# soedinglab/hh-suite

Measured on NVIDIA H100. Metric: Viterbi GCUPS (query_L x sum target_L / s), higher is better.
Workload: dtype f32

## Files before the change

### hh-suite_b200/csrc/hhg_api.cu

```cuda
#include "../../include/hhg.h"
#include "hhg_kernels.cuh"
#include "hhg_hhm.cuh"
#include "hhg_msa.cuh"
#include "hhg_crf.cuh"
#include "hhg_mac.cuh"
#include "hhg_topk.cuh"
#include "hhg_hitlist.h"

#include <dlfcn.h>
#if defined(__SSE__)
#include <xmmintrin.h>
#endif

#include <algorithm>
#include <chrono>
#include <atomic>
#include <cstdarg>
#include <cstdio>
#include <cstdlib>
#include <cstring>
#include <memory>
#include <cmath>
#include <cfloat>
#include <mutex>
// ... 1377 lines not shown
int hhg_set_use_ss(hhg_ctx* ctx, int use_ss) {
  if (!ctx) return fail(HHG_EINVAL, "ctx is NULL");
  if (use_ss && (!ctx->has_ss || !ctx->has_S33)) return fail(HHG_EINVAL, "hhg_set_use_ss: the query was set without ss / S33");
  ctx->par.use_ss = use_ss ? 1 : 0;
  return HHG_OK;
}

static int plan_strip_rows(const hhg_ctx* ctx, const int32_t* req_query, int n) {
  if (ctx->R) return ctx->R;
  long long items16 = 0;
  if (!req_query) items16 = (long long)((n + 31) / 32) * ((ctx->q_L[0] + 15) / 16);
  else {
    std::vector<long long> cnt(ctx->nq, 0);
    for (int k = 0; k < n; ++k) if (req_query[k] >= 0 && req_query[k] < ctx->nq) cnt[req_query[k]]++;
    for (int q = 0; q < ctx->nq; ++q) items16 += (cnt[q] + 31) / 32 * ((ctx->q_L[q] + 15) / 16);
  }
  return items16 >= 4LL * ctx->sm_count * 8 ? 16 : 8;
}

static int plan_build(hhg_ctx* ctx, hhg_plan* pl, const hhg_db* db, int n, const int32_t* ids,
                      const int32_t* req_query = nullptr) {
  if (!ctx || !db || n <= 0) return fail(HHG_EINVAL, "hhg_plan_create: bad argument");
  if (ctx->nq <= 0) return fail(HHG_EINVAL, "hhg_plan_create: no query set");
  if (db->device != ctx->device) return fail(HHG_EINVAL, "db lives on device %d, ctx on %d", db->device, ctx->device);
  CK(cudaSetDevice(ctx->device));
  const int R = plan_strip_rows(ctx, req_query, n);
  if (pl->db == db && pl->db_serial == db->serial && pl->n == n && pl->R == R && pl->q_L == ctx->q_L &&
      pl->q_row0 == ctx->q_row0 && !pl->ids.empty() && pl->max_bt_bytes == ctx->max_bt_bytes) {
    bool same = true;
    if (ids) same = memcmp(ids, pl->ids.data(), (size_t)n * 4) == 0;
    else for (int k = 0; k < n && same; ++k) same = pl->ids[k] == k;
    if (same) {
      if (req_query) same = memcmp(req_query, pl->req_query.data(), (size_t)n * 4) == 0;
      else for (int k = 0; k < n && same; ++k) same = pl->req_query[k] == 0;
    }
    if (same) { pl->celloff = false; return HHG_OK; }
  }
  pl->db = db;
  pl->db_serial = db->serial;
  pl->device = db->device;
  pl->max_bt_bytes = ctx->max_bt_bytes;
  pl->cells = pl->padded_cells = pl->alg_bytes = 0;
  pl->waves.clear();
  pl->celloff = false;
  pl->n = n;
  pl->R = R;
  pl->q_L = ctx->q_L; pl->q_row0 = ctx->q_row0;
  pl->Lq = ctx->q_L[0];
  pl->ids.resize(n); pl->req_query.resize(n);
  for (int k = 0; k < n; ++k) {
    const int id = ids ? ids[k] : k;
    if (id < 0 || id >= db->n) return fail(HHG_EINVAL, "request %d: target id %d out of range", k, id);
    const int q = req_query ? req_query[k] : 0;
    if (q < 0 || q >= ctx->nq) return fail(HHG_EINVAL, "request %d: query index %d out of range (batch of %d)", k, q, ctx->nq);
    pl->ids[k] = id; pl->req_query[k] = q;
  }
  pl->order.resize(n);
  std::iota(pl->order.begin(), pl->order.end(), 0);
  std::stable_sort(pl->order.begin(), pl->order.end(), [&](int a, int b) {
    if (pl->req_query[a] != pl->req_query[b]) return pl->req_query[a] < pl->req_query[b];
    return db->L[pl->ids[a]] > db->L[pl->ids[b]];
  });
  std::vector<int> job_first, job_cnt;
  for (int k = 0; k < n;) {
    const int q = pl->req_query[pl->order[k]];
    int e = k;
    while (e < n && e - k < 32 && pl->req_query[pl->order[e]] == q) ++e;
    job_first.push_back(k); job_cnt.push_back(e - k);
    k = e;
  }
  pl->njobs = (int)job_first.size();
  pl->req_job.resize(n); pl->req_lane.resize(n);
  pl->job_Lmax.resize(pl->njobs); pl->job_query.resize(pl->njobs); pl->job_nstrips.resize(pl->njobs);
  pl->job_Lq.resize(pl->njobs); pl->job_qrow0.resize(pl->njobs); pl->job_ss_off.resize(pl->njobs);
  pl->job_bt_off.resize(pl->njobs); pl->job_bnd_off.resize(pl->njobs); pl->job_co_off.resize(pl->njobs);
  pl->job_jc_off.resize(pl->njobs);
  pl->jc_version = 0;
  std::vector<int> job_target((size_t)pl->njobs * 32);
  std::vector<int> req_Lt(n), req_Lq(n);
  long long bnd = 0, co = 0, jc = 0, ss = 0;
  size_t wave_bt = 0, max_wave_words = 0;
  Wave w;
  for (int jb = 0; jb < pl->njobs; ++jb) {
    const int first = job_first[jb], cnt = job_cnt[jb];
    const int q = pl->req_query[pl->order[first]];
    const int Lmax = db->L[pl->ids[pl->order[first]]];
    const int ns = (ctx->q_L[q] + R - 1) / R;
    pl->job_Lmax[jb] = Lmax; pl->job_query[jb] = q; pl->job_nstrips[jb] = ns;
    pl->job_Lq[jb] = ctx->q_L[q]; pl->job_qrow0[jb] = ctx->q_row0[q];
    for (int l = 0; l < 32; ++l) {
      const int rq = pl->order[first + std::min(l, cnt - 1)];
      job_target[(size_t)jb * 32 + l] = pl->ids[rq];
      if (l < cnt) { pl->req_job[rq] = jb; pl->req_lane[rq] = l; }
    }
    const size_t words = (size_t)(ns * R / 4) * (Lmax + 1) * 32;
    if (wave_bt > 0 && (wave_bt + words) * 4 > ctx->max_bt_bytes) {
      w.job_end = jb;
      pl->waves.push_back(w);
      max_wave_words = std::max(max_wave_words, wave_bt);
      w.job_begin = jb;
      wave_bt = 0;
    }
    pl->job_bt_off[jb] = (long long)wave_bt;
    wave_bt += words;
    pl->job_bnd_off[jb] = bnd;
    bnd += (long long)(Lmax + 1) * 32;
    pl->job_co_off[jb] = co;
    pl->job_jc_off[jb] = jc;
    pl->job_ss_off[jb] = ss;
    jc += (long long)Lmax * 224;
    co += (long long)ns * (Lmax + 1) * 32;
    ss += ns;
    pl->padded_cells += (double)ns * R * (double)Lmax * 32.0;
  }
  w.job_end = pl->njobs;
  pl->waves.push_back(w);
  max_wave_words = std::max(max_wave_words, wave_bt);
  pl->ss_total = ss;
  pl->co_total = co;
  pl->items.clear();
  for (Wave& wv : pl->waves) {
    wv.item_begin = (long long)pl->items.size();
    for (int g0 = wv.job_begin; g0 < wv.job_end; g0 += ctx->group_jobs) {
      const int g1 = std::min(g0 + ctx->group_jobs, wv.job_end);
      int maxns = 0;
      for (int jb = g0; jb < g1; ++jb) maxns = std::max(maxns, pl->job_nstrips[jb]);
      for (int sidx = 0; sidx < maxns; ++sidx)
        for (int jb = g0; jb < g1; ++jb)
          if (sidx < pl->job_nstrips[jb]) pl->items.push_back(make_int2(jb - wv.job_begin, sidx));
    }
    wv.item_end = (long long)pl->items.size();
  }
  pl->path_off.resize(n);
  long long po = 0;
  double cols_sum = 0;
  for (int k = 0; k < n; ++k) {
    const int Lt = db->L[pl->ids[k]];
    const int Lqk = ctx->q_L[pl->req_query[k]];
    req_Lt[k] = Lt; req_Lq[k] = Lqk;
    pl->path_off[k] = po;
    po += Lqk + Lt + 2;
    pl->cells += (double)Lqk * Lt;
    cols_sum += Lt;
  }
  if (po > 0x7fffffffLL) return fail(HHG_EINVAL, "plan too large: %lld path bytes (> 2^31-1); split the request", po);
  pl->path_total = po;
  pl->jc_total = jc;
  pl->alg_bytes = cols_sum * 112.0 + pl->cells * 1.0 + (double)sizeof(HitRec) * n;

  cudaError_t e = cudaSuccess;
  auto A = [&](cudaError_t r) { if (e == cudaSuccess) e = r; };
  A(pl->d_job_target.ensure(job_target.size())); A(pl->d_job_Lmax.ensure(pl->njobs));
  A(pl->d_job_bt_off.ensure(pl->njobs)); A(pl->d_job_bnd_off.ensure(pl->njobs)); A(pl->d_job_co_off.ensure(pl->njobs));
  A(pl->d_job_jc_off.ensure(pl->njobs)); A(pl->d_jcols.ensure((size_t)jc + 224));
  A(pl->d_job_query.ensure(pl->njobs)); A(pl->d_job_nstrips.ensure(pl->njobs)); A(pl->d_job_Lq.ensure(pl->njobs));
  A(pl->d_job_qrow0.ensure(pl->njobs)); A(pl->d_job_ss_off.ensure(pl->njobs)); A(pl->d_items.ensure(pl->items.size()));
  A(pl->d_req_job.ensure(n)); A(pl->d_req_lane.ensure(n)); A(pl->d_req_Lt.ensure(n)); A(pl->d_req_Lq.ensure(n));
  A(pl->d_path_off.ensure(n));
  A(pl->d_req_target.ensure(n)); A(pl->d_S.ensure((size_t)po));
  A(pl->d_bt.ensure(max_wave_words));
  { BndSlot* before = pl->d_bnd.p; A(pl->d_bnd.ensure((size_t)bnd + 32));
    if (e == cudaSuccess && pl->d_bnd.p != before) A(cudaMemsetAsync(pl->d_bnd.p, 0, pl->d_bnd.n * sizeof(BndSlot), ctx->stream)); }
  A(pl->d_strip_score.ensure((size_t)ss * 32));
  A(pl->d_strip_ij.ensure((size_t)ss * 32));
  A(pl->d_counter.ensure(pl->waves.size()));
  A(pl->d_hits.ensure(n));
  A(pl->d_paths.ensure((size_t)po));
  if (e != cudaSuccess) return fail(HHG_ENOMEM, "hhg_plan_create: %s", cudaGetErrorString(e));

  cudaStream_t st = ctx->stream;
  auto H2D = [&](void* d, const void* h, size_t bytes) { return cudaMemcpyAsync(d, h, bytes, cudaMemcpyHostToDevice, st); };
  CK(H2D(pl->d_job_target.p, job_target.data(), job_target.size() * 4));
  CK(H2D(pl->d_job_Lmax.p, pl->job_Lmax.data(), (size_t)pl->njobs * 4));
  CK(H2D(pl->d_job_bt_off.p, pl->job_bt_off.data(), (size_t)pl->njobs * 8));
  CK(H2D(pl->d_job_bnd_off.p, pl->job_bnd_off.data(), (size_t)pl->njobs * 8));
  CK(H2D(pl->d_job_co_off.p, pl->job_co_off.data(), (size_t)pl->njobs * 8));
  CK(H2D(pl->d_job_jc_off.p, pl->job_jc_off.data(), (size_t)pl->njobs * 8));
  CK(H2D(pl->d_job_query.p, pl->job_query.data(), (size_t)pl->njobs * 4));
  CK(H2D(pl->d_job_nstrips.p, pl->job_nstrips.data(), (size_t)pl->njobs * 4));
  CK(H2D(pl->d_job_Lq.p, pl->job_Lq.data(), (size_t)pl->njobs * 4));
  CK(H2D(pl->d_job_qrow0.p, pl->job_qrow0.data(), (size_t)pl->njobs * 4));
  CK(H2D(pl->d_job_ss_off.p, pl->job_ss_off.data(), (size_t)pl->njobs * 8));
  CK(H2D(pl->d_items.p, pl->items.data(), pl->items.size() * sizeof(int2)));
  CK(H2D(pl->d_req_job.p, pl->req_job.data(), (size_t)n * 4));
  CK(H2D(pl->d_req_lane.p, pl->req_lane.data(), (size_t)n * 4));
  CK(H2D(pl->d_req_Lt.p, req_Lt.data(), (size_t)n * 4));
  CK(H2D(pl->d_req_Lq.p, req_Lq.data(), (size_t)n * 4));
  CK(H2D(pl->d_req_target.p, pl->ids.data(), (size_t)n * 4));
  CK(H2D(pl->d_path_off.p, pl->path_off.data(), (size_t)n * 8));
  CK(cudaStreamSynchronize(st));
  return HHG_OK;
}

int hhg_plan_create(hhg_ctx* ctx, const hhg_db* db, int n, const int32_t* ids, hhg_plan** out) {
  if (!out) return fail(HHG_EINVAL, "hhg_plan_create: out is NULL");
  std::unique_ptr<hhg_plan> pl(new hhg_plan());
  int rc = plan_build(ctx, pl.get(), db, n, ids);
  if (rc != HHG_OK) return rc;
  *out = pl.release();
  return HHG_OK;
}

int hhg_plan_destroy(hhg_plan* plan) {
  if (plan) { if (plan->db) cudaSetDevice(plan->device); delete plan; }
  return HHG_OK;
}
double hhg_plan_cells(const hhg_plan* plan) { return plan ? plan->cells : 0; }
double hhg_plan_padded_cells(const hhg_plan* plan) { return plan ? plan->padded_cells : 0; }
double hhg_plan_algorithmic_bytes(const hhg_plan* plan) { return plan ? plan->alg_bytes : 0; }

static int set_exclusions(hhg_ctx* ctx, hhg_plan* pl, const int64_t* excl_off, const int32_t* excl_i,
                          const int32_t* excl_j) {
  pl->celloff = false;
  pl->n_excl_steps = 0;
  const long long total = excl_off ? excl_off[pl->n] : 0;
  const bool regions = !ctx->ex_q_lo.empty() || !ctx->ex_t_lo.empty();
  if (total <= 0 && !regions) return HHG_OK;
  const size_t co_words = (size_t)pl->co_total;
  CK(pl->d_co.ensure(co_words));
  CK(cudaMemsetAsync(pl->d_co.p, 0, co_words * 4, ctx->stream));
  if (total > 0) {
    if (excl_off[0] != 0) return fail(HHG_EINVAL, "excl_off[0] must be 0");
    if (!excl_i || !excl_j) return fail(HHG_EINVAL, "excl_i / excl_j are NULL");
    std::vector<int> sreq((size_t)total);
    for (int k = 0; k < pl->n; ++k) {
      if (excl_off[k + 1] < excl_off[k]) return fail(HHG_EINVAL, "excl_off is not monotonic at request %d", k);
      const int Lt = pl->db->L[pl->ids[k]];
      for (long long s = excl_off[k]; s < excl_off[k + 1]; ++s) {
        const int Lqk = pl->q_L[pl->req_query[k]];
        if (excl_i[s] < 1 || excl_i[s] > Lqk || excl_j[s] < 1 || excl_j[s] > Lt)
          return fail(HHG_EINVAL, "excluded step %lld of request %d is (%d,%d), outside 1..%d x 1..%d", s - excl_off[k], k,
                      excl_i[s], excl_j[s], Lqk, Lt);
        sreq[(size_t)s] = k;
      }
    }
    CK(pl->d_step_req.ensure((size_t)total)); CK(pl->d_step_i.ensure((size_t)total)); CK(pl->d_step_j.ensure((size_t)total));
    CK(cudaMemcpyAsync(pl->d_step_req.p, sreq.data(), (size_t)total * 4, cudaMemcpyHostToDevice, ctx->stream));
    CK(cudaMemcpyAsync(pl->d_step_i.p, excl_i, (size_t)total * 4, cudaMemcpyHostToDevice, ctx->stream));
    CK(cudaMemcpyAsync(pl->d_step_j.p, excl_j, (size_t)total * 4, cudaMemcpyHostToDevice, ctx->stream));
    const int threads = 128;
    k_celloff_raster<<<(unsigned)((total + threads - 1) / threads), threads, 0, ctx->stream>>>(
        (int)total, pl->d_step_req.p, pl->d_step_i.p, pl->d_step_j.p, pl->d_req_job.p, pl->d_req_lane.p,
        pl->d_req_Lt.p, pl->d_req_Lq.p, pl->d_job_Lmax.p, pl->d_job_co_off.p, pl->R, pl->d_co.p);
    ctx->launches++;
    CK(cudaGetLastError());
    CK(cudaStreamSynchronize(ctx->stream));
  }
  if (regions) {
    const int nq = (int)ctx->ex_q_lo.size(), nt = (int)ctx->ex_t_lo.size();
    std::vector<int> h;
    h.insert(h.end(), ctx->ex_q_lo.begin(), ctx->ex_q_lo.end()); h.insert(h.end(), ctx->ex_q_hi.begin(), ctx->ex_q_hi.end());
    h.insert(h.end(), ctx->ex_t_lo.begin(), ctx->ex_t_lo.end()); h.insert(h.end(), ctx->ex_t_hi.begin(), ctx->ex_t_hi.end());
    CK(ctx->d_ex.ensure(h.size()));
    CK(cudaMemcpyAsync(ctx->d_ex.p, h.data(), h.size() * 4, cudaMemcpyHostToDevice, ctx->stream));
    const int* d = ctx->d_ex.p;
    k_celloff_regions<<<(unsigned)((co_words + 255) / 256), 256, 0, ctx->stream>>>(
        (long long)co_words, pl->njobs, pl->d_job_co_off.p, pl->d_job_Lmax.p, pl->d_job_nstrips.p, pl->R, nq, d, d + nq,
        nt, d + 2 * nq, d + 2 * nq + nt, pl->d_co.p);
    ctx->launches++;
    CK(cudaGetLastError());
    CK(cudaStreamSynchronize(ctx->stream));
  }
  pl->celloff = true;
  pl->n_excl_steps = (int)total;
  return HHG_OK;
}

int hhg_set_excluded_regions(hhg_ctx* ctx, int nq, const int32_t* q_lo, const int32_t* q_hi, int nt, const int32_t* t_lo,
                             const int32_t* t_hi) {
  if (!ctx || nq < 0 || nt < 0 || (nq && (!q_lo || !q_hi)) || (nt && (!t_lo || !t_hi)))
    return fail(HHG_EINVAL, "hhg_set_excluded_regions: bad argument");
  ctx->ex_q_lo.assign(q_lo, q_lo + nq); ctx->ex_q_hi.assign(q_hi, q_hi + nq);
  ctx->ex_t_lo.assign(t_lo, t_lo + nt); ctx->ex_t_hi.assign(t_hi, t_hi + nt);
  return HHG_OK;
}

}

template <int R>
static int launch_viterbi(hhg_ctx* ctx, const VitParams& P, bool local, bool ss, bool co, int items) {
  const size_t smem = (size_t)kWarpsPerCta * R * 112 + 64 + (ss ? 44 * 44 * 4 : 0);
  void (*kern)(const VitParams) = nullptr;
#define PICK(L_, S_, C_) kern = k_viterbi<R, L_, S_, C_>
  if (local) { if (ss) { if (co) PICK(true, true, true); else PICK(true, true, false); }
               else    { if (co) PICK(true, false, true); else PICK(true, false, false); } }
  else       { if (ss) { if (co) PICK(false, true, true); else PICK(false, true, false); }
               else    { if (co) PICK(false, false, true); else PICK(false, false, false); } }
#undef PICK
  CK(cudaFuncSetAttribute(kern, cudaFuncAttributeMaxDynamicSharedMemorySize, (int)smem));
  int per_sm = 0;
  CK(cudaOccupancyMaxActiveBlocksPerMultiprocessor(&per_sm, kern, kWarpsPerCta * 32, smem));
  if (per_sm < 1) return fail(HHG_ECUDA, "viterbi kernel does not fit on an SM");
  int grid = ctx->sm_count * per_sm;
  const int need = (items + kWarpsPerCta - 1) / kWarpsPerCta;
  if (grid > need) grid = need;
  kern<<<grid, kWarpsPerCta * 32, smem, ctx->stream>>>(P);
  ctx->launches++;
  CK(cudaGetLastError());
  return HHG_OK;
}

extern "C" {

static int plan_run_impl(hhg_ctx* ctx, hhg_plan* pl, bool timed) {
  if (!ctx || !pl) return fail(HHG_EINVAL, "hhg_plan_run: bad argument");
  if (pl->q_L != ctx->q_L || pl->q_row0 != ctx->q_row0) return fail(HHG_EINVAL, "plan was made for another query (batch) geometry");
  const hhg_db* db = pl->db;
  const bool fused = pl->nm_mode >= 0;
  if (fused && (!db->raw || !ctx->has_q_pav)) return fail(HHG_EINVAL, "fused null model needs a raw shard and query pav");
  if (!fused && !db->prepared) return fail(HHG_EINVAL, "raw db: call hhg_db_apply_null_model for the current query first");
  if (ctx->par.use_ss && (!db->has_ss || !ctx->has_ss || !ctx->has_S33))
    return fail(HHG_EINVAL, "use_ss requested but query/db/S33 carry no ss information");
  CK(cudaSetDevice(ctx->device));
  cudaStream_t st = ctx->stream;
  ctx->epoch = (ctx->epoch + 1) & 0xFFFFFu;
  if (ctx->epoch == 0) { ctx->epoch = 1; ctx->epoch_window++; }
  if (pl->bnd_epoch_window != ctx->epoch_window) {
    if (pl->d_bnd.p) CK(cudaMemsetAsync(pl->d_bnd.p, 0, pl->d_bnd.n * sizeof(BndSlot), st));
    pl->bnd_epoch_window = ctx->epoch_window;
  }
  CK(cudaMemsetAsync(pl->d_counter.p, 0, pl->waves.size() * 4, st));
  if (pl->jc_version != db->cols_version || pl->jc_nm_mode != pl->nm_mode ||
      (fused && pl->jc_query_serial != ctx->query_serial)) {
    int maxL = 0;
    for (int jb = 0; jb < pl->njobs; ++jb) maxL = std::max(maxL, pl->job_Lmax[jb]);
    dim3 grid((unsigned)pl->njobs, (unsigned)std::min(64, (maxL + 7) / 8), 1);
    k_interleave_cols<<<grid, 256, 0, st>>>(pl->njobs, pl->d_job_target.p, pl->d_job_Lmax.p, pl->d_job_jc_off.p,
                                            fused ? db->cols_raw.p : db->cols.p, db->dcol_off.p, db->dL.p, pl->d_jcols.p,
                                            pl->nm_mode, pl->d_job_query.p, ctx->d_q_pav.p, db->pav.p, ctx->d_pb.p);
    ctx->launches++;
    CK(cudaGetLastError());
    pl->jc_version = db->cols_version;
    pl->jc_nm_mode = pl->nm_mode;
    pl->jc_query_serial = ctx->query_serial;
  }
  for (size_t wi = 0; wi < pl->waves.size(); ++wi) {
    const Wave& w = pl->waves[wi];
    const int nj = w.job_end - w.job_begin;
    VitParams P{};
    P.qrec = ctx->qrec.p;
    P.job_Lq = pl->d_job_Lq.p + w.job_begin; P.job_nstrips = pl->d_job_nstrips.p + w.job_begin;
    P.job_qrow0 = pl->d_job_qrow0.p + w.job_begin; P.job_ss_off = pl->d_job_ss_off.p + w.job_begin;
    P.items = pl->d_items.p + w.item_begin; P.n_items = (int)(w.item_end - w.item_begin);
    P.Lt = db->dL.p;
    P.jcols = pl->d_jcols.p;
    P.job_jc_off = pl->d_job_jc_off.p + w.job_begin;
    P.njobs = nj;
    P.job_target = pl->d_job_target.p + (size_t)w.job_begin * 32;
    P.job_Lmax = pl->d_job_Lmax.p + w.job_begin;
    P.job_bt_off = pl->d_job_bt_off.p + w.job_begin;
    P.job_bnd_off = pl->d_job_bnd_off.p + w.job_begin;
    P.job_co_off = pl->d_job_co_off.p + w.job_begin;
    P.bt = pl->d_bt.p; P.bnd = pl->d_bnd.p;
    P.tag_base = ctx->epoch << 12;
    P.counter = pl->d_counter.p + wi;
    P.strip_score = pl->d_strip_score.p;
    P.strip_ij = pl->d_strip_ij.p;
    P.celloff = pl->celloff ? pl->d_co.p : nullptr;
    P.S33 = ctx->has_S33 ? ctx->S33.p : nullptr;
    P.egq = ctx->par.egq; P.egt = ctx->par.egt; P.shift = ctx->par.shift; P.ssw = ctx->par.ssw;
    P.zero = 0u;

    const int items = P.n_items;
    int rc;
    if (timed) CK(cudaEventRecord(ctx->ev[0], st));
    if (pl->R == 8) rc = launch_viterbi<8>(ctx, P, ctx->par.local != 0, ctx->par.use_ss != 0, pl->celloff, items);
    else if (pl->R == 12) rc = launch_viterbi<12>(ctx, P, ctx->par.local != 0, ctx->par.use_ss != 0, pl->celloff, items);
    else rc = launch_viterbi<16>(ctx, P, ctx->par.local != 0, ctx->par.use_ss != 0, pl->celloff, items);
    if (rc != HHG_OK) return rc;
    if (timed) CK(cudaEventRecord(ctx->ev[1], st));
    BtParams B{};
    B.n_req = pl->n;
    B.job_nstrips = pl->d_job_nstrips.p; B.job_ss_off = pl->d_job_ss_off.p; B.job_qrow0 = pl->d_job_qrow0.p;
    B.nm_mode = pl->nm_mode; B.job_query = pl->d_job_query.p; B.q_pav = ctx->d_q_pav.p; B.t_pav = db->pav.p;
    B.pb = ctx->d_pb.p;
    B.req_job = pl->d_req_job.p; B.req_lane = pl->d_req_lane.p;
    B.job_Lmax = pl->d_job_Lmax.p; B.job_bt_off = pl->d_job_bt_off.p;
    B.bt = pl->d_bt.p; B.strip_score = pl->d_strip_score.p; B.strip_ij = pl->d_strip_ij.p;
    B.path_off = pl->d_path_off.p; B.hits = pl->d_hits.p; B.paths = pl->d_paths.p;
    B.job_begin = w.job_begin; B.job_end = w.job_end;
    B.req_target = pl->d_req_target.p; B.qrec = ctx->qrec.p; B.cols = fused ? db->cols_raw.p : db->cols.p; B.col_off = db->dcol_off.p;
    B.lg2 = ctx->lg2.p; B.diff = ctx->diff.p; B.S33 = ctx->has_S33 ? ctx->S33.p : nullptr; B.S = pl->d_S.p;
    B.corr = ctx->par.corr; B.ssw = ctx->par.ssw; B.use_ss = ctx->par.use_ss; B.ss_score_mode = (ctx->par.ssm == 2);
    const int threads = 128;
    k_backtrace<<<(pl->n + threads - 1) / threads, threads, 0, st>>>(B);
    ctx->launches++;
    CK(cudaGetLastError());
    if (timed) {
      CK(cudaEventRecord(ctx->ev[2], st));
      CK(cudaEventSynchronize(ctx->ev[2]));
      float a = 0, b = 0;
      CK(cudaEventElapsedTime(&a, ctx->ev[0], ctx->ev[1]));
      CK(cudaEventElapsedTime(&b, ctx->ev[1], ctx->ev[2]));
      pl->ms_viterbi += a;
      pl->ms_backtrace += b;
    }
  }
  return HHG_OK;
}

int hhg_plan_run(hhg_ctx* ctx, hhg_plan* pl) { return plan_run_impl(ctx, pl, false); }

int hhg_plan_run_timed(hhg_ctx* ctx, hhg_plan* pl, float* ms_viterbi, float* ms_backtrace) {
  if (!ctx || !pl) return fail(HHG_EINVAL, "hhg_plan_run_timed: bad argument");
  for (int k = 0; k < 3; ++k)
    if (!ctx->ev[k]) CK(cudaEventCreate(&ctx->ev[k]));
  pl->ms_viterbi = pl->ms_backtrace = 0;
  int rc = plan_run_impl(ctx, pl, true);
  if (rc != HHG_OK) return rc;
  if (ms_viterbi) *ms_viterbi = pl->ms_viterbi;
  if (ms_backtrace) *ms_backtrace = pl->ms_backtrace;
  return HHG_OK;
}

int hhg_plan_fetch(hhg_ctx* ctx, hhg_plan* pl, hhg_hit* hits, uint8_t* paths, size_t paths_cap) {
  if (!ctx || !pl || !hits) return fail(HHG_EINVAL, "hhg_plan_fetch: bad argument");
  static_assert(sizeof(hhg_hit) == sizeof(HitRec), "hhg_hit / HitRec layout");
  CK(cudaSetDevice(ctx->device));
  CK(cudaMemcpyAsync(hits, pl->d_hits.p, (size_t)pl->n * sizeof(HitRec), cudaMemcpyDeviceToHost, ctx->stream));
  CK(cudaStreamSynchronize(ctx->stream));
  if (paths) {
    pl->h_compact_off.resize(pl->n);
    long long tot = 0;
    for (int k = 0; k < pl->n; ++k) { pl->h_compact_off[k] = tot; tot += hits[k].nsteps; }
    if (paths_cap < (size_t)tot) return fail(HHG_EINVAL, "paths buffer too small: need %lld bytes", tot);
    CK(pl->d_compact_off.ensure(pl->n));
    CK(pl->d_paths_compact.ensure((size_t)std::max<long long>(tot, 1)));
    CK(cudaMemcpyAsync(pl->d_compact_off.p, pl->h_compact_off.data(), (size_t)pl->n * 8, cudaMemcpyHostToDevice, ctx->stream));
    const int threads = 128;
    k_gather_paths<<<(pl->n + threads - 1) / threads, threads, 0, ctx->stream>>>(
        pl->n, pl->d_hits.p, pl->d_path_off.p, pl->d_compact_off.p, pl->d_paths.p, pl->d_paths_compact.p);
    ctx->launches++;
    CK(cudaGetLastError());
    CK(cudaMemcpyAsync(paths, pl->d_paths_compact.p, (size_t)tot, cudaMemcpyDeviceToHost, ctx->stream));
    CK(cudaStreamSynchronize(ctx->stream));
    for (int k = 0; k < pl->n; ++k) hits[k].path_off = (int32_t)pl->h_compact_off[k];
  }
  return HHG_OK;
}

void* hhg_plan_hits_devptr(hhg_plan* plan) { return plan ? (void*)plan->d_hits.p : nullptr; }
hhg_plan* hhg_ctx_last_plan(hhg_ctx* ctx) { return ctx ? ctx->scratch_plan : nullptr; }

int hhg_plan_debug_bt(hhg_ctx* ctx, hhg_plan* pl, int k, uint8_t* bt) {
  if (!ctx || !pl || !bt || k < 0 || k >= pl->n) return fail(HHG_EINVAL, "hhg_plan_debug_bt: bad argument");
  if (pl->waves.size() != 1) return fail(HHG_EINVAL, "debug_bt needs a single-wave plan");
  CK(cudaSetDevice(ctx->device));
  const int job = pl->req_job[k], lane = pl->req_lane[k];
  const int Lt = pl->db->L[pl->ids[k]];
  const int Lqk = pl->q_L[pl->req_query[k]];
  const int total = (Lqk + 1) * (Lt + 1);
  DevBuf<uint8_t> tmp;
  CK(tmp.alloc(total));
  k_debug_bt<<<(total + 255) / 256, 256, 0, ctx->stream>>>(pl->d_bt.p, pl->job_bt_off[job], lane,
                                                            pl->job_Lmax[job], Lqk, Lt, tmp.p);
  ctx->launches++;
  CK(cudaGetLastError());
  CK(cudaMemcpyAsync(bt, tmp.p, total, cudaMemcpyDeviceToHost, ctx->stream));
  CK(cudaStreamSynchronize(ctx->stream));
  return HHG_OK;
}

int hhg_viterbi_search(hhg_ctx* ctx, const hhg_db* db, int n, const int32_t* ids, hhg_hit* hits,
                       uint8_t* paths, size_t paths_cap, const int64_t* excl_off,
                       const int32_t* excl_i, const int32_t* excl_j) {
  if (!ctx) return fail(HHG_EINVAL, "ctx is NULL");
  if (!ctx->scratch_plan) ctx->scratch_plan = new hhg_plan();
  hhg_plan* pl = ctx->scratch_plan;
  static const bool timing = getenv("HHG_TIMING") != nullptr;
  auto now = [] { return std::chrono::steady_clock::now(); };
  auto t0 = now();
  int rc = plan_build(ctx, pl, db, n, ids);
  if (rc != HHG_OK) return rc;
  pl->nm_mode = -1;
  auto t1 = now();
  rc = set_exclusions(ctx, pl, excl_off, excl_i, excl_j);
  if (rc == HHG_OK) rc = hhg_plan_run(ctx, pl);
  if (timing) cudaStreamSynchronize(ctx->stream);
  auto t2 = now();
  if (rc == HHG_OK) rc = hhg_plan_fetch(ctx, pl, hits, paths, paths_cap);
  if (timing) {
    auto ms = [](decltype(t0) a, decltype(t0) b) { return std::chrono::duration<double, std::milli>(b - a).count(); };
    fprintf(stderr, "[hhg] viterbi_search n=%d: plan %.3f ms, run (device) %.3f ms, fetch %.3f ms\n", n, ms(t0, t1), ms(t1, t2), ms(t2, now()));
  }
  return rc;
}


int hhg_viterbi_search_batch(hhg_ctx* ctx, const hhg_db* db, int n, const int32_t* req_query, const int32_t* ids,
                             int columnscore, const float* pb, hhg_hit* hits, uint8_t* paths, size_t paths_cap) {
  if (!ctx || !db || !req_query || !ids) return fail(HHG_EINVAL, "hhg_viterbi_search_batch: bad argument");
  if (!ctx->scratch_plan) ctx->scratch_plan = new hhg_plan();
  hhg_plan* pl = ctx->scratch_plan;
  int rc = plan_build(ctx, pl, db, n, ids, req_query);
  if (rc != HHG_OK) return rc;
  pl->nm_mode = -1;
  if (db->raw) {
    if (columnscore < 0 || columnscore > 3) return fail(HHG_EINVAL, "hhg_viterbi_search_batch: columnscore %d", columnscore);
    if (!ctx->has_q_pav) return fail(HHG_EINVAL, "hhg_viterbi_search_batch: raw shard needs q_pav in hhg_query_set_batch");
    if (columnscore == 0 && !pb) return fail(HHG_EINVAL, "hhg_viterbi_search_batch: columnscore 0 needs pb");
    float h[20] = {0};
    if (pb) memcpy(h, pb, 80);
    CK(ctx->d_pb.ensure(20));
    CK(cudaMemcpyAsync(ctx->d_pb.p, h, 80, cudaMemcpyHostToDevice, ctx->stream));
    CK(cudaStreamSynchronize(ctx->stream));
    pl->nm_mode = columnscore;
  }
  rc = set_exclusions(ctx, pl, nullptr, nullptr, nullptr);
  if (rc == HHG_OK) rc = hhg_plan_run(ctx, pl);
  if (rc == HHG_OK) rc = hhg_plan_fetch(ctx, pl, hits, paths, paths_cap);
  return rc;
}

}
// ... 757 lines not shown
```

### hh-suite_b200/csrc/hhg_kernels.cuh

```cuda
#pragma once
#include <cuda_runtime.h>
#include <float.h>
#include <stdint.h>

#ifndef HHG_MAX3
#define HHG_MAX3 1
#endif

#include "hhg_math.cuh"

namespace hhg {

constexpr int kWarpsPerCta = 4;

struct __align__(16) ColRec {
  float p[20];
  float m2m, m2d, d2m, d2d, i2m;
  float i2i, m2i;
  uint32_t ss;
};
static_assert(sizeof(ColRec) == 112, "ColRec must be 7 x 16 bytes");

struct __align__(8) BndSlot {
  unsigned long long w[5];
};
static_assert(sizeof(BndSlot) == 40, "BndSlot must be five 64-bit words");

__device__ __forceinline__ unsigned long long tagged(float v, uint32_t tag) {
  return ((unsigned long long)tag << 32) | __float_as_uint(v);
}
__device__ __forceinline__ void st_slot(BndSlot* col, int lane, float mm, float dg, float mi, float gd, float im,
                                        uint32_t tag) {
  unsigned long long* p = reinterpret_cast<unsigned long long*>(col);
  asm volatile("st.relaxed.gpu.global.v2.b64 [%0], {%1,%2};" ::"l"(p + 2 * lane), "l"(tagged(mm, tag)),
               "l"(tagged(dg, tag)) : "memory");
  asm volatile("st.relaxed.gpu.global.v2.b64 [%0], {%1,%2};" ::"l"(p + 64 + 2 * lane), "l"(tagged(mi, tag)),
               "l"(tagged(gd, tag)) : "memory");
  asm volatile("st.relaxed.gpu.global.b64 [%0], %1;" ::"l"(p + 128 + lane), "l"(tagged(im, tag)) : "memory");
}
__device__ __forceinline__ void ld_slot(const BndSlot* col, int lane, float& mm, float& dg, float& mi, float& gd,
                                        float& im, uint32_t (&tag)[5]) {
  const unsigned long long* p = reinterpret_cast<const unsigned long long*>(col);
  unsigned long long w0, w1, w2, w3, w4;
  asm volatile("ld.relaxed.gpu.global.v2.b64 {%0,%1}, [%2];" : "=l"(w0), "=l"(w1) : "l"(p + 2 * lane) : "memory");
  asm volatile("ld.relaxed.gpu.global.v2.b64 {%0,%1}, [%2];" : "=l"(w2), "=l"(w3) : "l"(p + 64 + 2 * lane) : "memory");
  asm volatile("ld.relaxed.gpu.global.b64 %0, [%1];" : "=l"(w4) : "l"(p + 128 + lane) : "memory");
  mm = __uint_as_float((uint32_t)w0); tag[0] = (uint32_t)(w0 >> 32);
  dg = __uint_as_float((uint32_t)w1); tag[1] = (uint32_t)(w1 >> 32);
  mi = __uint_as_float((uint32_t)w2); tag[2] = (uint32_t)(w2 >> 32);
  gd = __uint_as_float((uint32_t)w3); tag[3] = (uint32_t)(w3 >> 32);
  im = __uint_as_float((uint32_t)w4); tag[4] = (uint32_t)(w4 >> 32);
}
__device__ __forceinline__ bool slot_ok(const uint32_t (&tag)[5], uint32_t want) {
  return ((tag[0] ^ want) | (tag[1] ^ want) | (tag[2] ^ want) | (tag[3] ^ want) | (tag[4] ^ want)) == 0u;
}

struct VitParams {
  const float4* qrec;
  const int* job_Lq;
  const int* job_nstrips;
  const int* job_qrow0;
  const long long* job_ss_off;
  const int2* items;
  int n_items;
  const int* Lt;
  const float4* jcols;
  const long long* job_jc_off;
  int njobs;
  const int* job_target;
  const int* job_Lmax;
  const long long* job_bt_off;
  const long long* job_bnd_off;
  uint32_t* bt;
  struct BndSlot* bnd;
  uint32_t tag_base;
  unsigned int* counter;
  float* strip_score;
  int* strip_ij;
  const uint32_t* celloff;
  const long long* job_co_off;
  const float* S33;
  float egq, egt, shift, ssw;
  uint32_t zero;
};

__device__ __forceinline__ uint32_t smem_u32(const void* p) {
  return static_cast<uint32_t>(__cvta_generic_to_shared(p));
}
__device__ __forceinline__ void mbar_init(uint64_t* bar, int count) {
  asm volatile("mbarrier.init.shared::cta.b64 [%0], %1;" ::"r"(smem_u32(bar)), "r"(count));
}
__device__ __forceinline__ void mbar_expect_tx(uint64_t* bar, uint32_t bytes) {
  asm volatile("mbarrier.arrive.expect_tx.shared::cta.b64 _, [%0], %1;" ::"r"(smem_u32(bar)), "r"(bytes)
               : "memory");
}
__device__ __forceinline__ void tma_bulk_g2s(void* dst, const void* src, uint32_t bytes, uint64_t* bar) {
  asm volatile(
      "cp.async.bulk.shared::cluster.global.mbarrier::complete_tx::bytes [%0], [%1], %2, [%3];" ::"r"(
          smem_u32(dst)),
      "l"(src), "r"(bytes), "r"(smem_u32(bar))
      : "memory");
}
__device__ __forceinline__ void mbar_wait(uint64_t* bar, uint32_t parity) {
  asm volatile(
      "{\n"
      ".reg .pred p;\n"
      "WAIT_LOOP:\n"
      "mbarrier.try_wait.parity.shared::cta.b64 p, [%0], %1;\n"
      "@p bra DONE;\n"
      "bra WAIT_LOOP;\n"
      "DONE:\n"
      "}\n" ::"r"(smem_u32(bar)),
      "r"(parity)
      : "memory");
}
__device__ __forceinline__ float log2f4_dev(float x) {
  const uint32_t u = __float_as_uint(x);
  const float e = __fadd_rn(__uint_as_float((u >> 23) | 0x4B000000u), -8388735.0f);
  const float m = __uint_as_float((u & 0x007FFFFFu) | 0x3F800000u);
  float p = -0.107254423828329604454f;
  p = __fadd_rn(__fmul_rn(p, m), 0.688243882994381274313f);
  p = __fadd_rn(__fmul_rn(p, m), -1.75647175389045657003f);
  p = __fadd_rn(__fmul_rn(p, m), 2.61761038894603480148f);
  p = __fmul_rn(p, __fadd_rn(m, -1.0f));
  return __fadd_rn(p, e);
}

__device__ __forceinline__ float dot20_dev(const float4 (&t)[5], const float4 (&q)[5]) {
  float r0 = __fmul_rn(t[0].x, q[0].x), r1 = __fmul_rn(t[0].y, q[0].y);
  float r2 = __fmul_rn(t[0].z, q[0].z), r3 = __fmul_rn(t[0].w, q[0].w);
#pragma unroll
  for (int m = 1; m < 5; ++m) {
    r0 = __fadd_rn(__fmul_rn(t[m].x, q[m].x), r0);
    r1 = __fadd_rn(__fmul_rn(t[m].y, q[m].y), r1);
    r2 = __fadd_rn(__fmul_rn(t[m].z, q[m].z), r2);
    r3 = __fadd_rn(__fmul_rn(t[m].w, q[m].w), r3);
  }
  return __fadd_rn(__fadd_rn(r0, r1), __fadd_rn(r2, r3));
}

__device__ __forceinline__ float4 ld_jc(const float4* p) { return __ldcg(p); }

#define HHG_NEG (-FLT_MAX)

template <int R, bool LOCAL, bool SS, bool CELLOFF>
__global__ void __launch_bounds__(kWarpsPerCta * 32, (R <= 12) ? 3 : 2)
    k_viterbi(const VitParams P) {
  static_assert(R % 4 == 0, "R must be a multiple of 4");
  extern __shared__ __align__(128) unsigned char smem_raw[];
  const int warp = threadIdx.x >> 5;
  const int lane = threadIdx.x & 31;
  float4* qs = reinterpret_cast<float4*>(smem_raw) + (size_t)warp * R * 7;
  constexpr size_t kBarOff = (size_t)kWarpsPerCta * R * 112;
  uint64_t* bars = reinterpret_cast<uint64_t*>(smem_raw + kBarOff);
  float* s33 = reinterpret_cast<float*>(smem_raw + kBarOff + 64);
  uint64_t* bar = bars + warp;

  if (lane == 0) mbar_init(bar, 1);
  if (SS) {
    for (int k = threadIdx.x; k < 44 * 44; k += blockDim.x) s33[k] = P.S33[k];
  }
  asm volatile("fence.mbarrier_init.release.cluster;" ::: "memory");
  __syncthreads();

  const float smin = LOCAL ? 0.0f : HHG_NEG;
  const int total_items = P.n_items;
  uint32_t parity = 0;

  for (;;) {
    int item = 0;
    if (lane == 0) item = (int)atomicAdd(P.counter, 1u);
    item = __shfl_sync(0xffffffffu, item, 0);
    if (item >= total_items) break;
    const int2 it = __ldg(P.items + item);
    const int job = it.x, s = it.y;
    const int Lq = P.job_Lq[job];
    const int nstrips = P.job_nstrips[job];
    const int i0 = s * R;

    if (lane == 0) {
      mbar_expect_tx(bar, R * 112);
      tma_bulk_g2s(qs, P.qrec + (size_t)(P.job_qrow0[job] + i0) * 7, R * 112, bar);
    }

    const int t = P.job_target[job * 32 + lane];
    const int Lt = P.Lt[t];
    const int Lmax = P.job_Lmax[job];
    const float4* jc = P.jcols + P.job_jc_off[job] + lane;
    const size_t bt_row_stride = (size_t)(Lmax + 1) * 32;
    uint32_t* btc = P.bt + P.job_bt_off[job] + lane + (size_t)(i0 >> 2) * bt_row_stride + 32;
    BndSlot* bndc = P.bnd + P.job_bnd_off[job] + 32;
    const uint32_t tag_in = P.tag_base + (uint32_t)s;
    const uint32_t tag_out = P.tag_base + (uint32_t)s + 1u;
    const bool last_strip = (s == nstrips - 1);
    const uint32_t* co = nullptr;
    if (CELLOFF) co = P.celloff + P.job_co_off[job] + (size_t)s * (Lmax + 1) * 32 + lane + 32;

    float MM[R], GD[R], IM[R], DG[R], Y[R];
#pragma unroll
    for (int r = 0; r < R; ++r) {
      MM[r] = __fmul_rn((float)(-(i0 + 1 + r)), P.egq);
      GD[r] = IM[r] = DG[r] = HHG_NEG;
    }
    float dtMM = __fmul_rn((float)(-i0), P.egq), dtDG = HHG_NEG, dtGD = HHG_NEG, dtIM = HHG_NEG;

    float best = HHG_NEG;
    int bi = 0, bj = 0;

    float4 nx[7];
#pragma unroll
    for (int k = 0; k < 7; ++k) nx[k] = ld_jc(jc + k * 32);

    float nMM = 0.f, nDG = 0.f, nMI = 0.f, nGD = 0.f, nIM = 0.f;
    uint32_t ntag[5] = {0u, 0u, 0u, 0u, 0u};
    if (s > 0) ld_slot(bndc, lane, nMM, nDG, nMI, nGD, nIM, ntag);

    mbar_wait(bar, parity);
    parity ^= 1u;
#pragma unroll
    for (int r = 0; r < R; ++r) Y[r] = __fadd_rn(HHG_NEG, qs[r * 7 + 5].x);

    for (int j = 1; j <= Lmax; ++j) {
      const float4 tp[5] = {nx[0], nx[1], nx[2], nx[3], nx[4]};
      const float t_m2m = nx[5].x, t_m2d = nx[5].y, t_d2m = nx[5].z, t_d2d = nx[5].w;
      const float t_i2m = nx[6].x, t_i2i = nx[6].y, t_m2i = nx[6].z;
      const uint32_t t_ss = __float_as_uint(nx[6].w);
      jc += 224;
#pragma unroll
      for (int k = 0; k < 7; ++k) nx[k] = ld_jc(jc + k * 32);

      float tMM, tDG, tMI, tGD, tIM;
      if (s == 0) {
        tMM = __fmul_rn((float)(-j), P.egt);
        tDG = tMI = tGD = tIM = HHG_NEG;
      } else {
        if (!__all_sync(0xffffffffu, slot_ok(ntag, tag_in))) {
          while (!slot_ok(ntag, tag_in)) {
            __nanosleep(20);
            ld_slot(bndc, lane, nMM, nDG, nMI, nGD, nIM, ntag);
          }
        }
        tMM = nMM; tDG = nDG; tMI = nMI; tGD = nGD; tIM = nIM;
        ld_slot(bndc + 32, lane, nMM, nDG, nMI, nGD, nIM, ntag);
      }
      uint32_t cow = 0;
      if (CELLOFF) cow = __ldg(co);

      float4 qa = qs[5], qb = qs[6];
      float pMM = __fadd_rn(dtMM, qa.x), pGD = __fadd_rn(dtGD, qa.x), pIM = __fadd_rn(dtIM, qb.x),
            pDG = __fadd_rn(dtDG, qa.z);
      float uMM = tMM, uDG = tDG, uMI = tMI;
      const float bcmp = (j <= Lt) ? best : INFINITY;
      float bc = bcmp;

      uint32_t word = SS ? 0u : (t_ss & P.zero);
#pragma unroll
      for (int r = 0; r < R; ++r) {
        float4 q[5];
#pragma unroll
        for (int k = 0; k < 5; ++k) q[k] = qs[r * 7 + k];
        const float q_m2m = qa.x, q_m2d = qa.y, q_d2m = qa.z, q_d2d = qa.w;
        const float q_i2m = qb.x, q_i2i = qb.y, q_m2i = qb.z;

        uint32_t b;
        float mm;
        const float c1 = __fadd_rn(pMM, t_m2m);
        const float c2 = __fadd_rn(pGD, t_d2m);
        const float c3 = __fadd_rn(pIM, t_m2m);
        const float c4 = __fadd_rn(pDG, t_m2m);
        const float c5 = __fadd_rn(Y[r], t_i2m);
#if HHG_MAX3
        mm = fmaxf(fmaxf(smin, c1), c2);
        mm = fmaxf(fmaxf(mm, c3), c4);
        mm = fmaxf(mm, c5);
        b = 6u;
        b = (c4 == mm) ? 5u : b;
        b = (c3 == mm) ? 4u : b;
        b = (c2 == mm) ? 3u : b;
        b = (c1 == mm) ? 2u : b;
        b = (smin == mm) ? 0u : b;
#else
        b = (c1 > smin) ? 2u : 0u; mm = fmaxf(smin, c1);
        b = (c2 > mm) ? 3u : b;    mm = fmaxf(mm, c2);
        b = (c3 > mm) ? 4u : b;    mm = fmaxf(mm, c3);
        b = (c4 > mm) ? 5u : b;    mm = fmaxf(mm, c4);
        b = (c5 > mm) ? 6u : b;    mm = fmaxf(mm, c5);
#endif

        float Si = log2f4_dev(dot20_dev(tp, q));
        if (SS) {
          const uint32_t q_ss = __float_as_uint(qb.w);
          Si = __fadd_rn(__fmul_rn(P.ssw, s33[q_ss * 44 + t_ss]), Si);
        }
        Si = __fadd_rn(Si, P.shift);
        mm = __fadd_rn(mm, Si);

        const float oMM = MM[r], oGD = GD[r], oIM = IM[r], oDG = DG[r];
        float a1, a2, gd, im, dg, mi;
        a1 = __fadd_rn(oMM, t_m2d); a2 = __fadd_rn(oGD, t_d2d);
        b |= (a1 > a2) ? 8u : 0u;  gd = fmaxf(a1, a2);
        a1 = __fadd_rn(__fadd_rn(oMM, q_m2i), t_m2m); a2 = __fadd_rn(__fadd_rn(oIM, q_i2i), t_m2m);
        b |= (a1 > a2) ? 16u : 0u; im = fmaxf(a1, a2);
        a1 = __fadd_rn(uMM, q_m2d); a2 = __fadd_rn(uDG, q_d2d);
        b |= (a1 > a2) ? 32u : 0u; dg = fmaxf(a1, a2);
        Y[r] = __fadd_rn(uMI, q_m2m);
        a1 = __fadd_rn(__fadd_rn(uMM, q_m2m), t_m2i); a2 = __fadd_rn(Y[r], t_i2i);
        b |= (a1 > a2) ? 64u : 0u; mi = fmaxf(a1, a2);

        if (CELLOFF) {
          const float off = ((cow >> r) & 1u) ? HHG_NEG : 0.0f;
          mm = __fadd_rn(mm, off); gd = __fadd_rn(gd, off); im = __fadd_rn(im, off);
          dg = __fadd_rn(dg, off); mi = __fadd_rn(mi, off);
        }

        word |= b << (8 * (r & 3));
        if ((r & 3) == 3) {
          __stcs(btc + (size_t)(r >> 2) * bt_row_stride, word);
          word = 0;
        }
        if (r + 1 < R) {
          qa = qs[(r + 1) * 7 + 5]; qb = qs[(r + 1) * 7 + 6];
          pMM = __fadd_rn(oMM, qa.x); pGD = __fadd_rn(oGD, qa.x); pIM = __fadd_rn(oIM, qb.x);
          pDG = __fadd_rn(oDG, qa.z);
        }
        uMM = mm; uDG = dg; uMI = mi;
        MM[r] = mm; GD[r] = gd; IM[r] = im; DG[r] = dg;
      }
      dtMM = tMM; dtDG = tDG; dtGD = tGD; dtIM = tIM;

      {
        float c0 = MM[0], c1 = MM[1], c2 = MM[2], c3 = MM[3];
#pragma unroll
        for (int r = 4; r < R; r += 4) {
          c0 = fmaxf(c0, MM[r]); c1 = fmaxf(c1, MM[r + 1]); c2 = fmaxf(c2, MM[r + 2]); c3 = fmaxf(c3, MM[r + 3]);
        }
        if (fmaxf(fmaxf(c0, c1), fmaxf(c2, c3)) >= bc) {
#pragma unroll
          for (int r = 0; r < R; ++r) {
            const float mm = MM[r];
            if (mm >= bc) {
              const int i = i0 + 1 + r;
              const bool cand = (i <= Lq) && (LOCAL || i == Lq || j == Lt);
              if (cand && (mm > best || i < bi)) { best = mm; bi = i; bj = j; bc = mm; }
            }
          }
        }
      }

      if (!last_strip) st_slot(bndc, lane, uMM, uDG, uMI, GD[R - 1], IM[R - 1], tag_out);
      bndc += 32;
      btc += 32;
      if (CELLOFF) co += 32;
    }
    const size_t o = ((size_t)P.job_ss_off[job] + s) * 32 + lane;
    P.strip_score[o] = best;
    P.strip_ij[o] = (bi << 16) | bj;
    __syncwarp();
  }
}

__device__ __forceinline__ void null_model_vec(int columnscore, const float* __restrict__ q_pav,
                                               const float* __restrict__ t_pav, const float* __restrict__ pb,
                                               float (&pn)[20]) {
#pragma unroll
  for (int a = 0; a < 20; ++a) {
    switch (columnscore) {
      case 0: pn[a] = pb[a]; break;
      case 2: pn[a] = t_pav[a]; break;
      case 3: pn[a] = q_pav[a]; break;
      default: pn[a] = __fmul_rn(0.5f, __fadd_rn(q_pav[a], t_pav[a])); break;
    }
  }
}
__device__ __forceinline__ float4 div4(float4 v, const float* pn) {
  v.x = __fdiv_rn(v.x, pn[0]); v.y = __fdiv_rn(v.y, pn[1]); v.z = __fdiv_rn(v.z, pn[2]); v.w = __fdiv_rn(v.w, pn[3]);
  return v;
}

struct HitRec {
  float score;
  int i2, j2, i1, j1, nsteps, matched_cols, path_off;
  float hit_score;
  float score_ss;
};

struct BtParams {
  int n_req;
  const int* job_nstrips;
  const long long* job_ss_off;
  const int* job_qrow0;
  int nm_mode;
  const int* job_query;
  const float* q_pav;
  const float* t_pav;
  const float* pb;
  int job_begin, job_end;
  const int* req_job;
  const int* req_lane;
  const int* job_Lmax;
  const long long* job_bt_off;
  const uint32_t* bt;
  const float* strip_score;
  const int* strip_ij;
  const long long* path_off;
  HitRec* hits;
  uint8_t* paths;
  const int* req_target;
  const float4* qrec;
  const float4* cols;
  const long long* col_off;
  const float* lg2;
  const float* diff;
  const float* S33;
  float* S;
  float corr, ssw;
  int use_ss;
  int ss_score_mode;
};

__device__ __forceinline__ float score_cols_dev(const float4* q, const float4* t, const float* lg2,
                                                const float* diff, const float* pn = nullptr) {
  float sum = 0.0f;
#pragma unroll
  for (int k = 0; k < 5; ++k) {
    const float4 a = q[k];
    const float4 b = pn ? div4(t[k], pn + 4 * k) : t[k];
    if (k == 0) sum = __fmul_rn(b.x, a.x); else sum = __fadd_rn(sum, __fmul_rn(b.x, a.x));
    sum = __fadd_rn(sum, __fmul_rn(b.y, a.y));
    sum = __fadd_rn(sum, __fmul_rn(b.z, a.z));
    sum = __fadd_rn(sum, __fmul_rn(b.w, a.w));
  }
  return fast_log2_dev(sum, lg2, diff);
}

__device__ __forceinline__ uint32_t bt_byte(const uint32_t* btj, size_t row_stride, int i, int j) {
  const uint32_t w = btj[(size_t)((i - 1) >> 2) * row_stride + (size_t)j * 32];
  return (w >> (8 * ((i - 1) & 3))) & 0xFFu;
}

__global__ void k_backtrace(const BtParams P) {
  const int k = blockIdx.x * blockDim.x + threadIdx.x;
  if (k >= P.n_req) return;
  const int job = P.req_job[k], lane = P.req_lane[k];
  if (job < P.job_begin || job >= P.job_end) return;
  float best = HHG_NEG;
  int ij = 0;
  const int nstrips = P.job_nstrips[job];
  for (int s = 0; s < nstrips; ++s) {
    const size_t o = ((size_t)P.job_ss_off[job] + s) * 32 + lane;
    const float v = P.strip_score[o];
    if (v > best) { best = v; ij = P.strip_ij[o]; }
  }
  const int i2 = ij >> 16, j2 = ij & 0xFFFF;
  const int Lmax = P.job_Lmax[job];
  const uint32_t* btj = P.bt + P.job_bt_off[job] + lane;
  const size_t rs = (size_t)(Lmax + 1) * 32;
  uint8_t* path = P.paths ? P.paths + P.path_off[k] : nullptr;

  const float4* tcol = P.cols + (size_t)P.col_off[P.req_target[k]] * 7;
  const float4* qrec = P.qrec + (size_t)P.job_qrow0[job] * 7;
  float pnv[20];
  const float* pn = nullptr;
  if (P.nm_mode >= 0) {
    null_model_vec(P.nm_mode, P.q_pav + (size_t)P.job_query[job] * 20, P.t_pav + (size_t)P.req_target[k] * 20, P.pb, pnv);
    pn = pnv;
  }
  float* S = P.S + P.path_off[k];
  float score_ss = 0.0f;

  int step = 0, i = i2, j = j2, mc = 0, li = i2, lj = j2;
  int state = 2;
  while (state != 0) {
    if (path) path[step] = (uint8_t)state;
    float Sv = 0.0f;
    if (state == 2 && i >= 1 && j >= 1) {
      Sv = score_cols_dev(qrec + (size_t)(i - 1) * 7, tcol + (size_t)(j - 1) * 7, P.lg2, P.diff, pn);
      if (P.use_ss) {
        const uint32_t qs = __float_as_uint(qrec[(size_t)(i - 1) * 7 + 6].w);
        const uint32_t ts = __float_as_uint(tcol[(size_t)(j - 1) * 7 + 6].w);
        score_ss = __fadd_rn(score_ss, __fmul_rn(P.ssw, P.S33[qs * 44 + ts]));
      }
    }
    S[step] = Sv;
    ++step;
    li = i; lj = j;
    const uint32_t c = (i >= 1 && j >= 1) ? bt_byte(btj, rs, i, j) : 0u;
    const int prev_state = state;
    switch (state) {
      case 2: ++mc; state = (i <= 1 || j <= 1) ? 0 : (int)(c & 7u); --i; --j; break;
      case 3: if (j <= 1) state = 0; else { if (c & 8u) state = 2; --j; } break;
      case 4: if (j <= 1) state = 0; else { if (c & 16u) state = 2; --j; } break;
      case 5: if (i <= 1) state = 0; else { if (c & 32u) state = 2; --i; } break;
      case 6: if (i <= 1) state = 0; else { if (c & 64u) state = 2; --i; } break;
      default: state = 0; break;
    }
    if (state == 0 && prev_state != 2 && li >= 1 && lj >= 1) {
      S[step - 1] = score_cols_dev(qrec + (size_t)(li - 1) * 7, tcol + (size_t)(lj - 1) * 7, P.lg2, P.diff, pn);
      if (P.use_ss) {
        const uint32_t qs = __float_as_uint(qrec[(size_t)(li - 1) * 7 + 6].w);
        const uint32_t ts = __float_as_uint(tcol[(size_t)(lj - 1) * 7 + 6].w);
        score_ss = __fadd_rn(score_ss, __fmul_rn(P.ssw, P.S33[qs * 44 + ts]));
      }
    }
  }
  if (path && step > 0) path[step - 1] = 2;
  float hs = best;
  if (P.ss_score_mode) hs = __fadd_rn(hs, -score_ss);
  float scorr = 0.0f;
  if (step > 0) {
// ... 345 lines not shown
```

Measured before the change: 177.9.

## Stream target columns into per-warp shared-memory ring via TMA bulk copies

Replaces per-lane register prefetch of the next target column from global memory with a per-warp shared-memory ring of four columns. Lane 0 fills it with bulk async copies, two columns per copy, tracked by mbarriers. This is meant to hide global load latency further ahead and free the registers that held the prefetched column. It costs much more shared memory per CTA, which may lower occupancy, and adds barrier waits and proxy fences. It also removes the padding read past the end of jcols and the unused P.zero trick.

```diff
diff --git a/hh-suite_b200/csrc/hhg_api.cu b/hh-suite_b200/csrc/hhg_api.cu
--- a/hh-suite_b200/csrc/hhg_api.cu
+++ b/hh-suite_b200/csrc/hhg_api.cu
@@ -1553,7 +1553,7 @@
   auto A = [&](cudaError_t r) { if (e == cudaSuccess) e = r; };
   A(pl->d_job_target.ensure(job_target.size())); A(pl->d_job_Lmax.ensure(pl->njobs));
   A(pl->d_job_bt_off.ensure(pl->njobs)); A(pl->d_job_bnd_off.ensure(pl->njobs)); A(pl->d_job_co_off.ensure(pl->njobs));
-  A(pl->d_job_jc_off.ensure(pl->njobs)); A(pl->d_jcols.ensure((size_t)jc + 224));
+  A(pl->d_job_jc_off.ensure(pl->njobs)); A(pl->d_jcols.ensure((size_t)jc));
   A(pl->d_job_query.ensure(pl->njobs)); A(pl->d_job_nstrips.ensure(pl->njobs)); A(pl->d_job_Lq.ensure(pl->njobs));
   A(pl->d_job_qrow0.ensure(pl->njobs)); A(pl->d_job_ss_off.ensure(pl->njobs)); A(pl->d_items.ensure(pl->items.size()));
   A(pl->d_req_job.ensure(n)); A(pl->d_req_lane.ensure(n)); A(pl->d_req_Lt.ensure(n)); A(pl->d_req_Lq.ensure(n));
@@ -1680,7 +1680,7 @@
 
 template <int R>
 static int launch_viterbi(hhg_ctx* ctx, const VitParams& P, bool local, bool ss, bool co, int items) {
-  const size_t smem = (size_t)kWarpsPerCta * R * 112 + 64 + (ss ? 44 * 44 * 4 : 0);
+  const size_t smem = vit_smem_bytes(R, ss);
   void (*kern)(const VitParams) = nullptr;
 #define PICK(L_, S_, C_) kern = k_viterbi<R, L_, S_, C_>
   if (local) { if (ss) { if (co) PICK(true, true, true); else PICK(true, true, false); }
@@ -1760,7 +1760,6 @@
     P.celloff = pl->celloff ? pl->d_co.p : nullptr;
     P.S33 = ctx->has_S33 ? ctx->S33.p : nullptr;
     P.egq = ctx->par.egq; P.egt = ctx->par.egt; P.shift = ctx->par.shift; P.ssw = ctx->par.ssw;
-    P.zero = 0u;
 
     const int items = P.n_items;
     int rc;
diff --git a/hh-suite_b200/csrc/hhg_kernels.cuh b/hh-suite_b200/csrc/hhg_kernels.cuh
--- a/hh-suite_b200/csrc/hhg_kernels.cuh
+++ b/hh-suite_b200/csrc/hhg_kernels.cuh
@@ -81,7 +81,6 @@
   const long long* job_co_off;
   const float* S33;
   float egq, egt, shift, ssw;
-  uint32_t zero;
 };
 
 __device__ __forceinline__ uint32_t smem_u32(const void* p) {
@@ -100,6 +99,9 @@
           smem_u32(dst)),
       "l"(src), "r"(bytes), "r"(smem_u32(bar))
       : "memory");
+}
+__device__ __forceinline__ void fence_proxy_async() {
+  asm volatile("fence.proxy.async.shared::cta;" ::: "memory");
 }
 __device__ __forceinline__ void mbar_wait(uint64_t* bar, uint32_t parity) {
   asm volatile(
@@ -139,7 +141,11 @@
   return __fadd_rn(__fadd_rn(r0, r1), __fadd_rn(r2, r3));
 }
 
-__device__ __forceinline__ float4 ld_jc(const float4* p) { return __ldcg(p); }
+constexpr int kRingCols = 4;
+constexpr int kColBytes = 7 * 32 * 16;
+__host__ __device__ constexpr size_t vit_smem_bytes(int R, bool ss) {
+  return (size_t)kWarpsPerCta * (kRingCols * kColBytes + R * 112) + 128 + (ss ? 44 * 44 * 4 : 0);
+}
 
 #define HHG_NEG (-FLT_MAX)
 
@@ -150,13 +156,20 @@
   extern __shared__ __align__(128) unsigned char smem_raw[];
   const int warp = threadIdx.x >> 5;
   const int lane = threadIdx.x & 31;
-  float4* qs = reinterpret_cast<float4*>(smem_raw) + (size_t)warp * R * 7;
-  constexpr size_t kBarOff = (size_t)kWarpsPerCta * R * 112;
-  uint64_t* bars = reinterpret_cast<uint64_t*>(smem_raw + kBarOff);
-  float* s33 = reinterpret_cast<float*>(smem_raw + kBarOff + 64);
-  uint64_t* bar = bars + warp;
-
-  if (lane == 0) mbar_init(bar, 1);
+  constexpr size_t kQsOff = (size_t)kWarpsPerCta * kRingCols * kColBytes;
+  constexpr size_t kBarOff = kQsOff + (size_t)kWarpsPerCta * R * 112;
+  static_assert(kRingCols == 4 && kWarpsPerCta * 3 * 8 <= 128, "ring = two halves of two columns; 128 B of barriers");
+  float4* ring = reinterpret_cast<float4*>(smem_raw) + (size_t)warp * kRingCols * 224;
+  float4* qs = reinterpret_cast<float4*>(smem_raw + kQsOff) + (size_t)warp * R * 7;
+  uint64_t* bar = reinterpret_cast<uint64_t*>(smem_raw + kBarOff) + warp * 3;
+  uint64_t* rbar = bar + 1;
+  float* s33 = reinterpret_cast<float*>(smem_raw + kBarOff + 128);
+
+  if (lane == 0) {
+    mbar_init(bar, 1);
+    mbar_init(rbar, 1);
+    mbar_init(rbar + 1, 1);
+  }
   if (SS) {
     for (int k = threadIdx.x; k < 44 * 44; k += blockDim.x) s33[k] = P.S33[k];
   }
@@ -166,6 +179,7 @@
   const float smin = LOCAL ? 0.0f : HHG_NEG;
   const int total_items = P.n_items;
   uint32_t parity = 0;
+  uint32_t rphase = 0;
 
   for (;;) {
     int item = 0;
@@ -186,7 +200,16 @@
     const int t = P.job_target[job * 32 + lane];
     const int Lt = P.Lt[t];
     const int Lmax = P.job_Lmax[job];
-    const float4* jc = P.jcols + P.job_jc_off[job] + lane;
+    const float4* jsrc = P.jcols + P.job_jc_off[job];
+    auto refill = [&](int h, int c) {
+      if (lane == 0) {
+        const uint32_t bytes = (c < Lmax ? 2u : 1u) * kColBytes;
+        mbar_expect_tx(rbar + h, bytes);
+        tma_bulk_g2s(ring + h * 448, jsrc + (size_t)(c - 1) * 224, bytes, rbar + h);
+      }
+    };
+    refill(0, 1);
+    if (Lmax >= 3) refill(1, 3);
     const size_t bt_row_stride = (size_t)(Lmax + 1) * 32;
     uint32_t* btc = P.bt + P.job_bt_off[job] + lane + (size_t)(i0 >> 2) * bt_row_stride + 32;
     BndSlot* bndc = P.bnd + P.job_bnd_off[job] + 32;
@@ -207,10 +230,6 @@
     float best = HHG_NEG;
     int bi = 0, bj = 0;
 
-    float4 nx[7];
-#pragma unroll
-    for (int k = 0; k < 7; ++k) nx[k] = ld_jc(jc + k * 32);
-
     float nMM = 0.f, nDG = 0.f, nMI = 0.f, nGD = 0.f, nIM = 0.f;
     uint32_t ntag[5] = {0u, 0u, 0u, 0u, 0u};
     if (s > 0) ld_slot(bndc, lane, nMM, nDG, nMI, nGD, nIM, ntag);
@@ -220,14 +239,14 @@
 #pragma unroll
     for (int r = 0; r < R; ++r) Y[r] = __fadd_rn(HHG_NEG, qs[r * 7 + 5].x);
 
-    for (int j = 1; j <= Lmax; ++j) {
-      const float4 tp[5] = {nx[0], nx[1], nx[2], nx[3], nx[4]};
-      const float t_m2m = nx[5].x, t_m2d = nx[5].y, t_d2m = nx[5].z, t_d2d = nx[5].w;
-      const float t_i2m = nx[6].x, t_i2i = nx[6].y, t_m2i = nx[6].z;
-      const uint32_t t_ss = __float_as_uint(nx[6].w);
-      jc += 224;
-#pragma unroll
-      for (int k = 0; k < 7; ++k) nx[k] = ld_jc(jc + k * 32);
+    auto column = [&](const int j, const float4* op) {
+      float4 tp[5];
+#pragma unroll
+      for (int k = 0; k < 5; ++k) tp[k] = op[k * 32];
+      const float4 o5 = op[5 * 32], o6 = op[6 * 32];
+      const float t_m2m = o5.x, t_m2d = o5.y, t_d2m = o5.z, t_d2d = o5.w;
+      const float t_i2m = o6.x, t_i2i = o6.y, t_m2i = o6.z;
+      const uint32_t t_ss = __float_as_uint(o6.w);
 
       float tMM, tDG, tMI, tGD, tIM;
       if (s == 0) {
@@ -253,7 +272,7 @@
       const float bcmp = (j <= Lt) ? best : INFINITY;
       float bc = bcmp;
 
-      uint32_t word = SS ? 0u : (t_ss & P.zero);
+      uint32_t word = 0;
 #pragma unroll
       for (int r = 0; r < R; ++r) {
         float4 q[5];
@@ -351,10 +370,26 @@
       bndc += 32;
       btc += 32;
       if (CELLOFF) co += 32;
+    };
+
+    for (int j = 1; j <= Lmax; ++j) {
+      const int h = ((j - 1) >> 1) & 1;
+      const bool second = ((j - 1) & 1) != 0;
+      if (!second) {
+        mbar_wait(rbar + h, (rphase >> h) & 1u);
+        rphase ^= 1u << h;
+      }
+      column(j, ring + (2 * h + (second ? 1 : 0)) * 224 + lane);
+      if (second && j + 3 <= Lmax) {
+        fence_proxy_async();
+        __syncwarp();
+        refill(h, j + 3);
+      }
     }
     const size_t o = ((size_t)P.job_ss_off[job] + s) * 32 + lane;
     P.strip_score[o] = best;
     P.strip_ij[o] = (bi << 16) | bj;
+    fence_proxy_async();
     __syncwarp();
   }
 }
```

Measured after the change: 182.6, median of 6. 2.7% higher.
